# isl-org/Open3D-ML

Measured on AMD Instinct MI355X. Metric: point-cloud frames/sec (RandLA-Net SemanticKITTI inference: H2D + kNN pyramid + forward), higher is better.
Workload: dtype f32

## Files before the change

### open3d-ml_amd/csrc/randla.hip

```cpp
#include <hip/hip_runtime.h>
#include <math.h>
#include <stdint.h>
#include <stdlib.h>

#include <type_traits>

#include "gemm.h"
#include <gfx950_ops.h>
#include "grid.h"
#include "ml3d_hip.h"

namespace ml3d {

static int64_t fuse_rows() {
#ifdef ML3D_TEST_HOOKS
    static const int64_t rows = [] { const char* e = getenv("ML3D_RANDLA_FUSE_ROWS"); return e ? (int64_t)atoll(e) : (int64_t)64 * 1024; }();
    return rows;
#else
    return 64 * 1024;
#endif
}

#ifndef ML3D_ATTN_B3
#define ML3D_ATTN_B3 3
// ... 110 lines not shown
        if (m0 + r < A.m_total) {
            float v = acc[r];
            if (A.act) v = lrelu(v, A.slope);
            A.out[(m0 + r) * A.cout + o] = v;
        }
    }
}

struct LfaArgs {
    const float* xyz;
    const int32_t* nidx;
    int64_t n, n0, m_total;
    const float* gfeat;
    const float* lse1_wt;
    const float* lse1_b;
    const float* lse2_wt;
    const float* lse2_b;
    const float* score_wt;
    const float* score_b;
    const float* pool_wt;
    const float* pool_b;
    const float* mlp2_wt;
    const float* mlp2_b;
    const float* short_wt;
    const float* short_b;
    const float* feat_in;
    int d_in;
    float* out;
    int64_t xcd_chunk;
    const float* gscore;
    const int32_t* order;
};

__device__ __forceinline__ int64_t xcd_tile(int64_t i, int xcd, int64_t chunk, int64_t tiles) {
    const int64_t ci = i / chunk;
    const int64_t c = ci * 8 + xcd;
    if (c * chunk >= tiles) return -1;
    return c * chunk + (i - ci * chunk);
}

static int64_t xcd_chunk_tiles(int64_t tiles, int64_t batch) {
    if (batch <= 0 || tiles < 64) return 0;
    int64_t nch = batch;
    while (nch < 32) nch *= 2;
    int64_t chunk = (tiles + nch - 1) / nch;
    return chunk > 0 ? chunk : 0;
}

template <int D>
struct LfaCfg {
    static constexpr int H = D / 2;
    static constexpr int TP = (LFA_THREADS / D) > 0 ? (LFA_THREADS / D) : 1;
    static constexpr int CPT = D > LFA_THREADS ? D / LFA_THREADS : 1;
    static constexpr int CT = D > LFA_THREADS ? LFA_THREADS : D;
    static constexpr int XSLAB = D * XROW + 4;
};

template <int D>
__device__ __forceinline__ float attentive_pool(const float* Xp, int c, const float* __restrict__ score_wt,
                                                float bias) {
    float acc[RK];
#pragma unroll
    for (int k = 0; k < RK; ++k) acc[k] = bias;
    for (int j = 0; j < D; ++j) {
        float w = score_wt[j * D + c];
        const float4* xr = reinterpret_cast<const float4*>(Xp + j * XROW);
#pragma unroll
        for (int q = 0; q < RK / 4; ++q) {
            float4 x = xr[q];
            acc[4 * q + 0] = fmaf(x.x, w, acc[4 * q + 0]);
            acc[4 * q + 1] = fmaf(x.y, w, acc[4 * q + 1]);
            acc[4 * q + 2] = fmaf(x.z, w, acc[4 * q + 2]);
            acc[4 * q + 3] = fmaf(x.w, w, acc[4 * q + 3]);
        }
    }
    float mx = acc[0];
#pragma unroll
    for (int k = 1; k < RK; ++k) mx = fmaxf(mx, acc[k]);
    float sum = 0.f, agg = 0.f;
// ... 2197 lines not shown
}

template <class F>
static int dispatch_width(int dd, F f) {
    switch (dd) {
        case 8: return f(std::integral_constant<int, 8>{});
        case 16: return f(std::integral_constant<int, 16>{});
        case 32: return f(std::integral_constant<int, 32>{});
        case 64: return f(std::integral_constant<int, 64>{});
        case 128: return f(std::integral_constant<int, 128>{});
        case 256: return f(std::integral_constant<int, 256>{});
        case 512: return f(std::integral_constant<int, 512>{});
        default: return ML3D_E_UNSUPPORTED;
    }
}

__global__ void __launch_bounds__(256)
gather_max(const float* __restrict__ feat, const int32_t* __restrict__ nidx, float* __restrict__ out,
           int64_t n_in, int64_t n_out, int64_t batch, int c) {
    int64_t e = (int64_t)blockIdx.x * blockDim.x + threadIdx.x;
    if (e >= batch * n_out * c) return;
    int ch = (int)(e % c);
    int64_t r = e / c;
    int64_t b = r / n_out, i = r - b * n_out;
    const int32_t* id = nidx + (b * n_in + i) * RK;
    float v = -__builtin_inff();
#pragma unroll
    for (int k = 0; k < RK; ++k) v = fmaxf(v, feat[(b * n_in + id[k]) * c + ch]);
    out[r * c + ch] = v;
}

__global__ void __launch_bounds__(256)
gather_max4(const float* __restrict__ feat, const int32_t* __restrict__ nidx, float* __restrict__ out, uint32_t n_in,
            uint32_t n_out, uint32_t cv , uint32_t rows_per_block, const int32_t* __restrict__ order) {
    const uint32_t rl = threadIdx.x / cv, q = threadIdx.x - rl * cv;
    const uint32_t j = blockIdx.x * rows_per_block + rl;
    if (rl >= rows_per_block || j >= n_out) return;
    const uint32_t b = blockIdx.y;
    const uint32_t i = order ? (uint32_t)order[(size_t)b * n_out + j] - b * n_out : j;
    const int32_t* id = nidx + ((size_t)b * n_in + i) * RK;
    const float4* base = reinterpret_cast<const float4*>(feat + (size_t)b * n_in * (4 * cv)) + q;
    const float ninf = -__builtin_inff();
    float4 v = make_float4(ninf, ninf, ninf, ninf);
#pragma unroll
    for (int k = 0; k < RK; ++k) {
        const float4 x = base[(uint32_t)id[k] * cv];
        v.x = fmaxf(v.x, x.x); v.y = fmaxf(v.y, x.y); v.z = fmaxf(v.z, x.z); v.w = fmaxf(v.w, x.w);
    }
    reinterpret_cast<float4*>(out + ((size_t)b * n_out + i) * (4 * cv))[q] = v;
}

__global__ void __launch_bounds__(256)
gather_max_adjoint(const float* __restrict__ feat, const int32_t* __restrict__ nidx, const float* __restrict__ gout,
                   float* __restrict__ gfeat, int64_t n_in, int64_t n_out, int64_t batch, int c) {
    const int64_t e = (int64_t)blockIdx.x * blockDim.x + threadIdx.x;
    if (e >= batch * n_out * c) return;
    const int ch = (int)(e % c);
    const int64_t r = e / c;
    const int64_t b = r / n_out, i = r - b * n_out;
    const int32_t* id = nidx + (b * n_in + i) * RK;
    int64_t arg = b * n_in + id[0];
    float v = feat[arg * c + ch];
#pragma unroll
    for (int k = 1; k < RK; ++k) {
        const int64_t row = b * n_in + id[k];
        const float x = feat[row * c + ch];
        if (x > v) { v = x; arg = row; }
    }
    atomicAdd(gfeat + arg * c + ch, gout[r * c + ch]);
}

constexpr int AP_KMAX = 32;
template <bool BWD>
__global__ void __launch_bounds__(256)
attentive_pool_k(const float* __restrict__ scores, const float* __restrict__ x, const float* __restrict__ out_saved,
                 const float* __restrict__ gout, int64_t rows, int k, int c, float* __restrict__ out,
                 float* __restrict__ gscores, float* __restrict__ gx) {
    const int64_t e = (int64_t)blockIdx.x * blockDim.x + threadIdx.x;
    if (e >= rows * c) return;
    const int ch = (int)(e % c);
    const int64_t r = e / c;
    const float* sp = scores + r * k * c + ch;
// ... 291 lines not shown
            LfaArgs q1 = s1; q1.out = agg;
            const bool epi16 = dd == 16 && d_in == 8;
            if (epi16) q1.out = p1;
            const bool split = dd >= 32 && dd <= 256 && M * dd * 4 < ((int64_t)1 << 32) && M < ((int64_t)1 << 30);
            const bool b3_attn = ((ML3D_ATTN_B3) & 1) != 0 && split && ((dd == 128 && n[l] >= B3Cfg<128, 1>::TP) || (dd == 256 && n[l] >= B3Cfg<256, 1>::TP));
            auto point_scores = [&](const float* gfeat, int score_w, int score_b) {
                return run(8 * l + 7, lin(gfeat, h, score_w, (dd <= 64 || b3_attn) ? score_b : -1, p2, M, dd, 0.f));
            };
            if (split) { rc = point_scores(f1, sb + 4, sb + 5); if (rc) return rc; q1.gscore = p2; }
            rc = T.traced(8 * l + 1, [&] {
                return dispatch_width(dd, [&](auto w) { return launch_attn<decltype(w)::value, 1>(q1, st, epi16); });
            });
            if (rc) return rc;
            if (!epi16) {
                rc = run(8 * l + 4, lin(agg, dd, sb + 6, sb + 7, p1, M, h, 0.2f));
                if (rc) return rc;
            }
            LfaArgs q2 = s2; q2.out = epi16 ? enc : agg;
            if (split) { rc = point_scores(p1, sb + 10, sb + 11); if (rc) return rc; q2.gscore = p2; }
            rc = T.traced(8 * l + 2, [&] {
                return dispatch_width(dd, [&](auto w) { return launch_attn<decltype(w)::value, 2>(q2, st, epi16); });
            });
            if (rc) return rc;
            if (!epi16) {
                const LinArgs pool2[2] = {lin(agg, dd, sb + 12, sb + 13, p2, M, dd, 0.2f),
                                          lin(p2, dd, sb + 14, sb + 16, enc, M, 2 * dd, 0.01f, feat, d_in, sb + 17)};
                rc = launch_linears(pool2, 2, M >= fuse_rows(), T, 8 * l + 5, st);
            }
        } else {
            rc = dispatch_width(dd, [&](auto w) { return launch_lfa<decltype(w)::value>(s1, s2, st, T, 8 * l + 1); });
        }
        if (rc) return rc;
        rc = T.traced(8 * l + 3, [&] {
            const int c2 = 2 * dd;
            if ((c2 & 3) == 0 && c2 / 4 <= 256 && n[l] * c2 < ((int64_t)1 << 32) && B < 65536) {
                const uint32_t cv = (uint32_t)(c2 / 4), rpb = 256u / cv;
                const int32_t* ord = (tile_order && l + 1 < Lr) ? tile_order[l + 1] : nullptr;
                hipLaunchKernelGGL(gather_max4, dim3((unsigned)((n[l + 1] + rpb - 1) / rpb), (unsigned)B), dim3(256), 0, st, enc,
                                   neighbor_idx[l], samp, (uint32_t)n[l], (uint32_t)n[l + 1], cv, rpb, ord);
            } else {
                const int64_t items = B * n[l + 1] * c2;
                hipLaunchKernelGGL(gather_max, dim3((unsigned)((items + 255) / 256)), dim3(256), 0, st, enc,
                                   neighbor_idx[l], samp, n[l], n[l + 1], B, c2);
            }
            return hipGetLastError() == hipSuccess ? 0 : ML3D_E_LAUNCH;
        });
        if (rc) return rc;
        if (l == 0) enc_keep[0] = enc;
        enc_keep[l + 1] = samp;
        feat = samp;
        d_in = 2 * dd;
    }
    int slot = 2 + 18 * Lr;
    const int Dm = d_in;
    float* cur = take(B * n[Lr] * Dm);
    rc = run(1001, lin(feat, Dm, slot, slot + 1, cur, B * n[Lr], Dm, 0.2f));
    if (rc) return rc;
    slot += 2;
    auto fc1 = [&, fs = slot + 2 * Lr](LinArgs* g, const float* in, int k, float* t0, float* t1) {
        g[0] = lin(in, k, fs, fs + 1, t0, B * n[0], 64, 0.2f);
        g[1] = lin(t0, 64, fs + 2, fs + 3, t1, B * n[0], 32, 0.2f);
        g[2] = lin(t1, 32, fs + 4, fs + 5, out_scores, B * n[0], d->num_classes, 0.f);
    };
    int ed[ML3D_RANDLA_MAX_LAYERS + 1];
    enc_dims(d, ed);
    int cprev = Dm;
    for (int i = 0; i < Lr; ++i) {
        const int lev = Lr - 1 - i;
        const int skip_c = ed[Lr + 1 - i - 2];
        float* outp = take(B * n[lev] * skip_c);
        LinArgs a = lin(enc_keep[Lr + 1 - i - 2], skip_c, slot, slot + 1, outp, B * n[lev], skip_c, 0.2f, cur, cprev);
        a.gather = interp_idx[lev]; a.rows_per_item = n[lev]; a.a1_rows_per_item = n[lev + 1];
        if (i == Lr - 1) {
            LinArgs g[4] = {a};
            fc1(g + 1, outp, skip_c, nullptr, nullptr);
            const ChainArgs ch = chain_of(g, 4);
            if (mlp_shape_matches<ShapeDecFc1>(ch)) return T.traced(1200, [&] { return launch_chain_auto(ch, st); });
        }
        if (n[lev] >= 64 && (skip_c & 3) == 0 && (cprev & 3) == 0 && skip_c >= 8) {
            float* up = take(B * n[lev + 1] * skip_c);
            rc = T.traced(1100 + i, [&] {
                RowsA Au = {};
                Au.a = cur; Au.lda = cprev; Au.k1 = cprev;
                const int r = gemm_rows(Au, a.wt + (int64_t)skip_c * skip_c, B * n[lev + 1], skip_c, cprev, Epilogue{}, up, skip_c, nullptr, 0, st);
                if (r) return r;
                RowsA As = {};
                As.a = a.a0; As.lda = skip_c; As.k1 = skip_c;
                const Epilogue e1 = Epilogue::of(a.bias, 1, 0.2f).residual_rows(up, skip_c).gathered_residual(a.gather, 0, n[lev + 1], n[lev], n[lev + 1]);
                return gemm_rows(As, a.wt, a.m_total, skip_c, skip_c, e1, outp, skip_c, nullptr, 0, st);
            });
        } else {
            rc = run(1100 + i, a);
        }
        if (rc) return rc;
        slot += 2;
        cur = outp;
        cprev = skip_c;
    }
    float* t0 = take(B * n[0] * 64);
    float* t1 = take(B * n[0] * 32);
    LinArgs g[3];
    fc1(g, cur, cprev, t0, t1);
    return launch_linears(g, 3, true, T, 1200, st);
}

extern "C" int ml3d_randla_gather_max(const float* features, const int32_t* pool_idx, int64_t batch, int64_t n_in, int64_t n_out,
                                      int channels, float* out, void* stream) {
    if (batch < 0 || n_in < 0 || n_out < 0 || n_out > n_in || channels <= 0) return ML3D_E_INVALID;
    if (batch * n_out == 0) return 0;
    if (!features || !pool_idx || !out) return ML3D_E_INVALID;
    const int64_t total = batch * n_out * channels;
    hipLaunchKernelGGL(gather_max, dim3((unsigned)((total + 255) / 256)), dim3(256), 0, (hipStream_t)stream, features, pool_idx, out,
                       n_in, n_out, batch, channels);
    return hipGetLastError() == hipSuccess ? 0 : ML3D_E_LAUNCH;
}

extern "C" int ml3d_randla_gather_max_backward(const float* features, const int32_t* pool_idx, const float* grad_out, int64_t batch,
                                               int64_t n_in, int64_t n_out, int channels, float* grad_features, void* stream) {
    if (batch < 0 || n_in < 0 || n_out < 0 || n_out > n_in || channels <= 0) return ML3D_E_INVALID;
    if (batch * n_in == 0) return 0;
    if (!grad_features) return ML3D_E_INVALID;
    hipStream_t st = (hipStream_t)stream;
    if (hipMemsetAsync(grad_features, 0, sizeof(float) * (size_t)(batch * n_in) * (size_t)channels, st) != hipSuccess) return ML3D_E_LAUNCH;
    if (n_out == 0) return 0;
    if (!features || !pool_idx || !grad_out) return ML3D_E_INVALID;
    const int64_t total = batch * n_out * channels;
    hipLaunchKernelGGL(gather_max_adjoint, dim3((unsigned)((total + 255) / 256)), dim3(256), 0, st, features, pool_idx, grad_out,
                       grad_features, n_in, n_out, batch, channels);
    return hipGetLastError() == hipSuccess ? 0 : ML3D_E_LAUNCH;
}

extern "C" int ml3d_randla_attentive_pool(const float* scores, const float* x, int64_t rows, int k, int channels, float* out,
                                          void* stream) {
    if (rows < 0 || k <= 0 || channels <= 0) return ML3D_E_INVALID;
    if (k > AP_KMAX) return ML3D_E_UNSUPPORTED;
    if (rows == 0) return 0;
    if (!scores || !x || !out) return ML3D_E_INVALID;
    const int64_t total = rows * channels;
    hipLaunchKernelGGL((attentive_pool_k<false>), dim3((unsigned)((total + 255) / 256)), dim3(256), 0, (hipStream_t)stream, scores, x,
                       nullptr, nullptr, rows, k, channels, out, nullptr, nullptr);
    return hipGetLastError() == hipSuccess ? 0 : ML3D_E_LAUNCH;
}

extern "C" int ml3d_randla_attentive_pool_backward(const float* scores, const float* x, const float* out, const float* grad_out,
                                                   int64_t rows, int k, int channels, float* grad_scores, float* grad_x,
                                                   void* stream) {
    if (rows < 0 || k <= 0 || channels <= 0) return ML3D_E_INVALID;
// ... 9 lines not shown
```

### open3d-ml_amd/csrc/grid.h

```cpp
#pragma once
#include <hip/hip_runtime.h>
#include <stdint.h>

namespace ml3d {

constexpr int GRID_CAP = 8;
constexpr int GRID_SLACK = 64;
constexpr int GRID_LEVELS = 5;

struct Segs {
    const int64_t* splits;
    int64_t stride;
    int64_t n_uniform;
    int batch;
};

struct GridSeg {
    float lo[3];
    float c, inv_c;
    float margin;
    int dims[3];
    int cell_base;
    int n;
    int sorted_base;
    float c0;
    int dims0[3];
    float ext[3];
    float dim_est;
    int probe_stride;
};

struct GridView {
    const GridSeg* segs;
    const int* cell_start;
    const float4* sorted;
    int batch;
};

struct GridWs {
    GridSeg* segs;
    unsigned* bbox;
    unsigned* occ;
    unsigned* bitmap;
    int* cells;
    int* block_sums;
    float4* sorted;
    int64_t total_cells;
    int64_t bitmap_words;
    int64_t n_total;
    int batch;
};

constexpr int GRID_SORTED_SLACK = 4;
size_t grid_ws_bytes(int64_t n_total, int64_t batch);
bool grid_ws_carve(void* ws, size_t bytes, int64_t n_total, int64_t batch, GridWs* out);
int grid_build(const float* points, Segs segs, const GridWs& ws, float target_occ, hipStream_t stream);
int grid_build_derived(const float* points, Segs segs, const GridWs& ws, const GridWs& parent, hipStream_t stream);
int grid_build_fixed(const float* points, Segs segs, const GridWs& ws, float cell, hipStream_t stream);
int bbox_compute(const float* points, Segs segs, int64_t n_total, unsigned* bbox, unsigned* occ_scratch,
                 hipStream_t stream);
int scan_inclusive_i32(int* a, int64_t n, int* block_sums, hipStream_t stream);

void zero_async(void* ptr, size_t bytes, hipStream_t stream);

static inline char* ws_align(void* ws) { return (char*)(((uintptr_t)ws + 255) & ~(uintptr_t)255); }
static inline size_t ws_avail(const void* ws, size_t bytes) { return ws && bytes > 256 ? bytes - 256 : 0; }

__device__ __forceinline__ unsigned f2ord(float f) {
    unsigned u = __float_as_uint(f);
    return (u & 0x80000000u) ? ~u : (u | 0x80000000u);
}
__device__ __forceinline__ float ord2f(unsigned u) {
    return __uint_as_float((u & 0x80000000u) ? (u & 0x7fffffffu) : ~u);
}

__device__ __forceinline__ void wave_sync() {
    __threadfence_block();
    __builtin_amdgcn_wave_barrier();
}

__device__ __forceinline__ void wave_lds_sync() {
    __builtin_amdgcn_fence(__ATOMIC_RELEASE, "wavefront");
    __builtin_amdgcn_wave_barrier();
    __builtin_amdgcn_fence(__ATOMIC_ACQUIRE, "wavefront");
}


__device__ __forceinline__ float fmax_raw(float a, float b) { return __builtin_amdgcn_fmed3f(a, b, 3.0e38f); }

__device__ __forceinline__ int wave_inclusive_scan(int v) {
// ... 95 lines not shown
```

### open3d-ml_amd/csrc/grid.hip

```cpp
#include "grid.h"

#include <math.h>

namespace ml3d {

static inline size_t align_up(size_t x) { return (x + 255) & ~(size_t)255; }

static void grid_sizes(int64_t n_total, int64_t batch, int64_t* total_cells, int64_t* bitmap_words,
                       int64_t* n_blocks) {
    *total_cells = (int64_t)GRID_CAP * n_total + (int64_t)GRID_SLACK * batch;
    *bitmap_words = (*total_cells + 31) / 32 + batch;
    *n_blocks = (*total_cells + 2 + 1023) / 1024 + 1;
}

size_t grid_ws_bytes(int64_t n_total, int64_t batch) {
    int64_t tc, bw, nb;
    grid_sizes(n_total, batch, &tc, &bw, &nb);
    size_t b = 0;
    b += align_up(sizeof(GridSeg) * (size_t)batch);
    b += align_up(sizeof(unsigned) * 6 * (size_t)batch);
    b += align_up(sizeof(unsigned) * GRID_LEVELS * (size_t)batch);
    b += align_up(sizeof(unsigned) * GRID_LEVELS * (size_t)bw);
    b += align_up(sizeof(int) * (size_t)(tc + 2));
    b += align_up(sizeof(int) * (size_t)nb);
// ... 427 lines not shown
    for (int r = 0; r < 16; ++r) {
        int incl = wave_inclusive_scan(v[r]) + carry;
        int64_t i = base + r * 64 + lane;
        if (i < n) a[i] = incl;
        carry = __shfl(incl, 63);
    }
}

constexpr int SCAN_ONE_MAX = 32768;

__global__ void __launch_bounds__(1024) scan_one(int* a, int n) {
    __shared__ int ws[16];
    const int lane = threadIdx.x & 63, wv = threadIdx.x >> 6;
    const int rows = (n + 1023) / 1024;
    const int base = wv * rows * 64;
    int tot = 0;
    for (int r = 0; r < rows; ++r) {
        const int i = base + r * 64 + lane;
        if (i < n) tot += a[i];
    }
    tot = wave_sum(tot);
    if (lane == 0) ws[wv] = tot;
    __syncthreads();
    int carry = 0;
    for (int w = 0; w < wv; ++w) carry += ws[w];
    for (int r = 0; r < rows; ++r) {
        const int i = base + r * 64 + lane;
        const int incl = wave_inclusive_scan(i < n ? a[i] : 0) + carry;
        if (i < n) a[i] = incl;
        carry = __shfl(incl, 63);
    }
}

__global__ void grid_scatter(const float* __restrict__ pts, Segs S, int64_t n_total,
                             const GridSeg* __restrict__ segs, int* cells, float4* sorted) {
    int64_t i = (int64_t)blockIdx.x * blockDim.x + threadIdx.x;
    if (i >= n_total) return;
    int s; int64_t local;
    seg_locate(S, i, s, local);
    const float* p = pts + 3 * (seg_begin_global(S, s) + local);
    float x = p[0], y = p[1], z = p[2];
    int cid = point_cell(&segs[s], x, y, z);
    int pos = atomicAdd(&cells[cid + 1], 1);
    sorted[pos] = make_float4(x, y, z, __int_as_float((int)local));
}

__global__ void __launch_bounds__(256) grid_zero(uint4* __restrict__ p, size_t n16, uint32_t* __restrict__ tail, int ntail) {
    const size_t i = (size_t)blockIdx.x * blockDim.x + threadIdx.x;
    const size_t step = (size_t)gridDim.x * blockDim.x;
    for (size_t j = i; j < n16; j += step) p[j] = make_uint4(0u, 0u, 0u, 0u);
    if (i < (size_t)ntail) tail[i] = 0u;
}

void zero_async(void* ptr, size_t bytes, hipStream_t stream) {
    if (bytes == 0) return;
    if ((((uintptr_t)ptr) & 15) || (bytes & 3)) { (void)hipMemsetAsync(ptr, 0, bytes, stream); return; }
    const size_t n16 = bytes / 16;
    const int ntail = (int)((bytes - 16 * n16) / 4);
    const size_t want = (n16 + 255) / 256;
    const unsigned nb = (unsigned)(want < 1 ? 1 : (want > 2048 ? 2048 : want));
    hipLaunchKernelGGL(grid_zero, dim3(nb), dim3(256), 0, stream, (uint4*)ptr, n16, (uint32_t*)((char*)ptr + 16 * n16), ntail);
}

#define ML3D_LAUNCH_CHECK()                         \
    do {                                            \
        if (hipGetLastError() != hipSuccess) return -3; \
    } while (0)

int scan_inclusive_i32(int* a, int64_t n, int* block_sums, hipStream_t stream) {
    if (n <= 0) return 0;
    if (n <= SCAN_ONE_MAX) {
        hipLaunchKernelGGL(scan_one, dim3(1), dim3(1024), 0, stream, a, (int)n);
        ML3D_LAUNCH_CHECK();
        return 0;
    }
    int sbk = (int)((n + SCAN_TILE - 1) / SCAN_TILE);
    hipLaunchKernelGGL(scan_block_sums, dim3(sbk), dim3(256), 0, stream, a, n, block_sums);
    ML3D_LAUNCH_CHECK();
    hipLaunchKernelGGL(scan_sums, dim3(1), dim3(1024), 0, stream, block_sums, (int64_t)sbk);
    ML3D_LAUNCH_CHECK();
    hipLaunchKernelGGL(scan_final, dim3(sbk), dim3(256), 0, stream, a, n, block_sums);
    ML3D_LAUNCH_CHECK();
    return 0;
}

static int grid_sort(const float* points, Segs S, const GridWs& ws, hipStream_t stream) {
    int64_t n = ws.n_total;
    int nb = (int)((n + 255) / 256);
    if (n > 0) {
        hipLaunchKernelGGL(grid_hist, dim3(nb), dim3(256), 0, stream, points, S, n, ws.segs, ws.cells);
        ML3D_LAUNCH_CHECK();
        if (scan_inclusive_i32(ws.cells + 2, ws.total_cells, ws.block_sums, stream)) return -3;
        hipLaunchKernelGGL(grid_scatter, dim3(nb), dim3(256), 0, stream, points, S, n, ws.segs, ws.cells,
                           ws.sorted);
        ML3D_LAUNCH_CHECK();
    }
    return 0;
}


int grid_build(const float* points, Segs S, const GridWs& ws, float target_occ, hipStream_t stream) {
    int64_t n = ws.n_total;
    int B = ws.batch;
    if (B <= 0) return 0;
    if (target_occ <= 0.f) target_occ = 4.0f;
    int sb = (B + 63) / 64;
    zero_async(ws.bitmap, (size_t)((char*)(ws.cells + ws.total_cells + 2) - (char*)ws.bitmap), stream);
    hipLaunchKernelGGL(grid_bbox_init, dim3(sb), dim3(64), 0, stream, ws.bbox, ws.occ, B);
    ML3D_LAUNCH_CHECK();
    if (n > 0) {
        int nb4 = (int)((n + 1023) / 1024);
        hipLaunchKernelGGL(grid_bbox, dim3(nb4), dim3(256), 0, stream, points, S, n, ws.bbox);
        ML3D_LAUNCH_CHECK();
    }
    hipLaunchKernelGGL(grid_setup0, dim3(sb), dim3(64), 0, stream, S, ws.bbox, ws.segs, B);
    ML3D_LAUNCH_CHECK();
    int nb = (int)((n + 255) / 256);
    if (n > 0) {
        const int dense = (!S.splits && S.n_uniform >= 32768) ? 16 : 0;
        const int nbo = dense ? (int)((((S.n_uniform + dense - 1) / dense) * (int64_t)S.batch + 255) / 256) : nb;
        hipLaunchKernelGGL(grid_occupancy, dim3(nbo), dim3(256), 0, stream, points, S, n, ws.segs, ws.bitmap,
                           ws.bitmap_words, ws.occ, dense);
        ML3D_LAUNCH_CHECK();
    }
    hipLaunchKernelGGL(grid_setup1, dim3(sb), dim3(64), 0, stream, ws.occ, ws.segs, B, target_occ);
    ML3D_LAUNCH_CHECK();
    return grid_sort(points, S, ws, stream);
}

__global__ void grid_setup_fixed(GridSeg* segs, int batch, float cell) {
    int s = blockIdx.x * blockDim.x + threadIdx.x;
    if (s >= batch) return;
    GridSeg g = segs[s];
    float c = cell;
    if (!(c > 0.f)) c = g.c0;
    if (c < g.c0 * 0.5f) c = g.c0 * 0.5f;
    finish_grid(g, c, (int64_t)GRID_CAP * g.n + GRID_SLACK);
    segs[s] = g;
}

int bbox_compute(const float* points, Segs S, int64_t n, unsigned* bbox, unsigned* occ_scratch, hipStream_t stream) {
    int B = S.batch;
    if (B <= 0) return 0;
    hipLaunchKernelGGL(grid_bbox_init, dim3((B + 63) / 64), dim3(64), 0, stream, bbox, occ_scratch, B);
    ML3D_LAUNCH_CHECK();
    if (n > 0) {
        hipLaunchKernelGGL(grid_bbox, dim3((unsigned)((n + 1023) / 1024)), dim3(256), 0, stream, points, S, n, bbox);
        ML3D_LAUNCH_CHECK();
    }
    return 0;
}

int grid_build_fixed(const float* points, Segs S, const GridWs& ws, float cell, hipStream_t stream) {
    int B = ws.batch;
    if (B <= 0) return 0;
    int sb = (B + 63) / 64;
    zero_async(ws.cells, sizeof(int) * (size_t)(ws.total_cells + 2), stream);
    if (bbox_compute(points, S, ws.n_total, ws.bbox, ws.occ, stream)) return -3;
    hipLaunchKernelGGL(grid_setup0, dim3(sb), dim3(64), 0, stream, S, ws.bbox, ws.segs, B);
    ML3D_LAUNCH_CHECK();
    hipLaunchKernelGGL(grid_setup_fixed, dim3(sb), dim3(64), 0, stream, ws.segs, B, cell);
    ML3D_LAUNCH_CHECK();
    return grid_sort(points, S, ws, stream);
}

int grid_build_derived(const float* points, Segs S, const GridWs& ws, const GridWs& parent, hipStream_t stream) {
    int B = ws.batch;
    if (B <= 0) return 0;
    zero_async(ws.cells, sizeof(int) * (size_t)(ws.total_cells + 2), stream);
    hipLaunchKernelGGL(grid_setup_derived, dim3((B + 63) / 64), dim3(64), 0, stream, S, parent.segs, ws.segs, B);
    ML3D_LAUNCH_CHECK();
    return grid_sort(points, S, ws, stream);
}

}
```

### open3d-ml_amd/csrc/knn.hip

```cpp
#include <hip/hip_runtime.h>
#include <stdint.h>
#include <stdlib.h>

#include <gfx950_ops.h>

#include "grid.h"
#include "ml3d_hip.h"

namespace ml3d {

typedef unsigned long long u64;
constexpr u64 KEY_EMPTY = 0x7ff0000000000000ull;

struct QuerySrc {
    const float4* sorted_q;
    const GridSeg* qsegs;
    const float* raw;
    Segs segs;
    int64_t n_total;
};

template <int K>
__device__ __forceinline__ void topk_insert(double (&best)[K], double key) {
    if (key < best[K - 1]) {
// ... 324 lines not shown
        hipLaunchKernelGGL((knn_first<16, SUB>), dim3(blocks), dim3(T), 0, stream, J, k, index_local, vec, H);
        if (hipGetLastError() != hipSuccess) return ML3D_E_LAUNCH;
        hipLaunchKernelGGL((knn_continue<16, SUB>), dim3((H.cap + T - 1) / T), dim3(T), 0, stream, J, k, index_local, vec, H);
        return hipGetLastError() == hipSuccess ? 0 : ML3D_E_LAUNCH;
    }
    if (k == 1) hipLaunchKernelGGL((knn_query_multi<1, SUB, false>), dim3(blocks), dim3(T), 0, stream, J, k, index_local, vec, H);
    else if (k <= 8) hipLaunchKernelGGL((knn_query_multi<8, SUB, false>), dim3(blocks), dim3(T), 0, stream, J, k, index_local, vec, H);
    else if (k <= 16) hipLaunchKernelGGL((knn_query_multi<16, SUB, false>), dim3(blocks), dim3(T), 0, stream, J, k, index_local, vec, H);
    else if (k <= 32) hipLaunchKernelGGL((knn_query_multi<32, SUB, false>), dim3(blocks), dim3(T), 0, stream, J, k, index_local, vec, H);
    else if (k <= 64) hipLaunchKernelGGL((knn_query_multi<64, SUB, false>), dim3(blocks), dim3(T), 0, stream, J, k, index_local, vec, H);
    else return ML3D_E_UNSUPPORTED;
    return hipGetLastError() == hipSuccess ? 0 : ML3D_E_LAUNCH;
}

static int launch_query(const GridView& G, const QuerySrc& Q, int k, int index_local, Segs support_segs,
                        int32_t* out_idx, float* out_d2, hipStream_t stream) {
    if (Q.n_total <= 0) return 0;
    dim3 grid((unsigned)((Q.n_total + 255) / 256)), block(256);
    if (k == 1)
        hipLaunchKernelGGL(knn_query<1>, grid, block, 0, stream, G, Q, k, index_local, support_segs, out_idx, out_d2);
    else if (k <= 8)
        hipLaunchKernelGGL(knn_query<8>, grid, block, 0, stream, G, Q, k, index_local, support_segs, out_idx, out_d2);
    else if (k <= 16)
        hipLaunchKernelGGL(knn_query<16>, grid, block, 0, stream, G, Q, k, index_local, support_segs, out_idx, out_d2);
    else if (k <= 32)
        hipLaunchKernelGGL(knn_query<32>, grid, block, 0, stream, G, Q, k, index_local, support_segs, out_idx, out_d2);
    else if (k <= 64)
        hipLaunchKernelGGL(knn_query<64>, grid, block, 0, stream, G, Q, k, index_local, support_segs, out_idx, out_d2);
    else
        return ML3D_E_UNSUPPORTED;
    return hipGetLastError() == hipSuccess ? 0 : ML3D_E_LAUNCH;
}

__global__ void order_from_grid(const float4* __restrict__ sorted, int64_t n_total, int64_t n_per_item,
                                int32_t* __restrict__ out) {
    const int64_t i = (int64_t)blockIdx.x * blockDim.x + threadIdx.x;
    if (i >= n_total) return;
    out[i] = (int32_t)((i / n_per_item) * n_per_item + (int64_t)__float_as_int(sorted[i].w));
}

static constexpr float tuning_occ() { return 0.f; }

}

using namespace ml3d;

extern "C" int ml3d_abi_version(void) { return ML3D_ABI_VERSION; }

extern "C" size_t ml3d_knn_workspace_bytes(int64_t n_points, int64_t n_queries, int64_t batch) {
    (void)n_queries;
    return grid_ws_bytes(n_points, batch);
}

extern "C" int ml3d_knn_search(const float* points, const int64_t* points_row_splits, const float* queries,
                               const int64_t* queries_row_splits, int64_t batch, int64_t n_points,
                               int64_t n_queries, int k, int index_local, int32_t* out_index,
                               float* out_dist2, void* workspace, size_t workspace_bytes, void* stream) {
    if (!points_row_splits || !queries_row_splits || batch <= 0 || k <= 0 || n_points < 0 || n_queries < 0 ||
        n_points > 0x7fffffffll / GRID_CAP - 4096 || n_queries > 0x7fffffffll)
        return ML3D_E_INVALID;
    if (k > 64) return ML3D_E_UNSUPPORTED;
    if (n_queries == 0) return 0;
    if (!out_index || (n_points > 0 && !points) || !queries) return ML3D_E_INVALID;
    GridWs ws;
    if (!grid_ws_carve(workspace, workspace_bytes, n_points, batch, &ws)) return ML3D_E_WORKSPACE;
    hipStream_t st = (hipStream_t)stream;
    Segs ps = {points_row_splits, 0, 0, (int)batch};
    Segs qs = {queries_row_splits, 0, 0, (int)batch};
    int rc = grid_build(points, ps, ws, tuning_occ(), st);
    if (rc) return ML3D_E_LAUNCH;
    GridView G = grid_view(ws);
    QuerySrc Q;
    bool self = (queries == points) && (queries_row_splits == points_row_splits) && (n_queries == n_points);
// ... 41 lines not shown
    return ml3d_randla_knn_pyramid_ordered(points, batch, n0, num_layers, ratios_host, k, neighbor_idx_host,
                                           interp_idx_host, nullptr, workspace, workspace_bytes, stream, tr);
}

extern "C" int ml3d_randla_knn_pyramid_ordered(const float* points, int64_t batch, int64_t n0, int num_layers,
                                               const int32_t* ratios_host, int k,
                                               int32_t* const* neighbor_idx_host, int32_t* const* interp_idx_host,
                                               int32_t* const* tile_order_host, void* workspace,
                                               size_t workspace_bytes, void* stream, const ml3d_trace* tr) {
    auto tb = [&](int tag) { for (const ml3d_trace* r = tr; r; r = r->next) if (r->tag == tag && r->ev_start) (void)hipEventRecord((hipEvent_t)r->ev_start, (hipStream_t)stream); };
    auto te = [&](int tag) { for (const ml3d_trace* r = tr; r; r = r->next) if (r->tag == tag && r->ev_stop) (void)hipEventRecord((hipEvent_t)r->ev_stop, (hipStream_t)stream); };
    if (!points || batch <= 0 || n0 <= 0 || num_layers <= 0 || num_layers > KNN_MAX_JOBS || !ratios_host || k <= 0 ||
        !neighbor_idx_host || !interp_idx_host)
        return ML3D_E_INVALID;
    if (k > 64) return ML3D_E_UNSUPPORTED;
    int64_t n[17];
    if (pyramid_sizes(n0, num_layers, ratios_host, n)) return ML3D_E_INVALID;
    if (n0 * batch > 0x7fffffffll / GRID_CAP - 4096) return ML3D_E_INVALID;
    if (workspace_bytes < ml3d_randla_pyramid_workspace_bytes(batch, n0, num_layers, ratios_host))
        return ML3D_E_WORKSPACE;
    hipStream_t st = (hipStream_t)stream;
    GridWs ws[17];
    char* p = (char*)workspace;
    for (int l = 0; l < num_layers; ++l) {
        size_t bytes = grid_ws_bytes(n[l] * batch, batch) + 256;
        if (!grid_ws_carve(p, bytes, n[l] * batch, batch, &ws[l])) return ML3D_E_WORKSPACE;
        p += bytes;
    }
    float occ = tuning_occ();
    for (int l = 0; l < num_layers; ++l) {
        if (n[l] == 0) continue;
        Segs S = {nullptr, n0, n[l], (int)batch};
        tb(100 + l);
        if (l == 0 ? grid_build(points, S, ws[l], occ, st) : grid_build_derived(points, S, ws[l], ws[0], st))
            return ML3D_E_LAUNCH;
        if (tile_order_host && tile_order_host[l]) {
            const int64_t nt = n[l] * batch;
            hipLaunchKernelGGL(order_from_grid, dim3((unsigned)((nt + 255) / 256)), dim3(256), 0, st, ws[l].sorted, nt, n[l],
                               tile_order_host[l]);
            if (hipGetLastError() != hipSuccess) return ML3D_E_LAUNCH;
        }
        te(100 + l);
    }
    KnnJobs Jk;
    Jk.n = 0;
    for (int l = 0; l < num_layers; ++l) {
        if (n[l] == 0) continue;
        Segs S = {nullptr, n0, n[l], (int)batch};
        QuerySrc Q;
        Q.sorted_q = ws[l].sorted;
        Q.qsegs = ws[l].segs;
        Q.raw = points;
        Q.segs = S;
        Q.n_total = n[l] * batch;
        KnnJob& a = Jk.j[Jk.n++];
        a.G = grid_view(ws[l]); a.Q = Q; a.support = S; a.out_idx = neighbor_idx_host[l]; a.block_begin = 0;
        a.out_sub = interp_idx_host[l];
        a.n_sub = (int)n[l + 1];
    }
    int64_t total_q = 0;
    for (int l = 0; l < num_layers; ++l) total_q += n[l] * batch;
    const Handoff hand = handoff_carve(p, total_q);
    tb(0);
    int rc = launch_query_multi<true>(Jk, k, 1, st, &hand);
    te(0);
    return rc;
}

#include <hip/hip_fp16.h>

#include "patchloop.h"
#include "sort.h"

namespace ml3d {
// ... 248 lines not shown
```

Before: 7474.

## Split pooling gather into L2-sized channel slabs with XCD-aware block mapping

The random-sampling max-pool gather now divides the channel dimension into slabs sized so that one slab of the input feature map fits in a 2 MiB L2 budget. Blocks are remapped so that each XCD processes contiguous chunks of a single (batch, slab) unit. The aim is to keep gathered neighbour rows resident in each XCD's L2 rather than re-reading them from HBM. The public gather_max entry point also moves to the vectorised path when alignment allows. This adds index arithmetic per block, and narrower slabs make each thread's loads less contiguous.

After: 7496 (median of 2 runs). About the same (+0.3%).

```diff
diff --git a/open3d-ml_amd/csrc/randla.hip b/open3d-ml_amd/csrc/randla.hip
--- a/open3d-ml_amd/csrc/randla.hip
+++ b/open3d-ml_amd/csrc/randla.hip
@@ -166,9 +166,10 @@
     const int32_t* order;
 };
 
-__device__ __forceinline__ int64_t xcd_tile(int64_t i, int xcd, int64_t chunk, int64_t tiles) {
-    const int64_t ci = i / chunk;
-    const int64_t c = ci * 8 + xcd;
+template <class I>
+__device__ __forceinline__ I xcd_tile(I i, int xcd, I chunk, I tiles) {
+    const I ci = i / chunk;
+    const I c = ci * 8 + xcd;
     if (c * chunk >= tiles) return -1;
     return c * chunk + (i - ci * chunk);
 }
@@ -179,6 +180,30 @@
     while (nch < 32) nch *= 2;
     int64_t chunk = (tiles + nch - 1) / nch;
     return chunk > 0 ? chunk : 0;
+}
+
+constexpr int64_t POOL_L2_BUDGET = (int64_t)2 << 20;
+struct PoolPlan {
+    int w;
+    int rpb;
+    int64_t chunk, split;
+    unsigned grid;
+};
+static PoolPlan pool_plan(int64_t B, int64_t n_in, int64_t n_out, int c, bool ordered) {
+    const PoolPlan plain = {c, 256 / (c / 4), 0, 1, 0};
+    int w = c;
+    if (c % 32 == 0 && c > 32) {
+        w = 32;
+        for (int x = 64; x <= c; x += 32)
+            if (c % x == 0 && n_in * x * 4 <= POOL_L2_BUDGET) w = x;
+    }
+    const int64_t slabs = c / w, rpb = 256 / (w / 4), rb = (n_out + rpb - 1) / rpb;
+    if (B * slabs < 8 || (ordered && c <= 32)) return plain;
+    int64_t split = 1;
+    while (B * slabs * split < 32) split *= 2;
+    const int64_t chunk = (rb + split - 1) / split, nch = B * slabs * split;
+    if (nch * chunk + 8 * chunk >= ((int64_t)1 << 31)) return plain;
+    return PoolPlan{w, (int)rpb, chunk, split, (unsigned)(8 * ((nch + 7) / 8 * chunk))};
 }
 
 template <int D>
@@ -2442,14 +2467,24 @@
 
 __global__ void __launch_bounds__(256)
 gather_max4(const float* __restrict__ feat, const int32_t* __restrict__ nidx, float* __restrict__ out, uint32_t n_in,
-            uint32_t n_out, uint32_t cv , uint32_t rows_per_block, const int32_t* __restrict__ order) {
-    const uint32_t rl = threadIdx.x / cv, q = threadIdx.x - rl * cv;
-    const uint32_t j = blockIdx.x * rows_per_block + rl;
+            uint32_t n_out, uint32_t cv , uint32_t wv , uint32_t rows_per_block,
+            const int32_t* __restrict__ order, uint32_t batch, int32_t xcd_chunk, int32_t split) {
+    const uint32_t rl = threadIdx.x / wv, q = threadIdx.x - rl * wv;
+    uint32_t b = blockIdx.y, jb = blockIdx.x, q0 = 0;
+    if (xcd_chunk > 0) {
+        const int32_t rb = (int32_t)((n_out + rows_per_block - 1) / rows_per_block);
+        const int32_t per_cs = split * xcd_chunk, slabs = (int32_t)(cv / wv), units = (int32_t)batch * slabs * per_cs;
+        const int32_t t = xcd_tile<int32_t>((int32_t)(blockIdx.x >> 3), (int)(blockIdx.x & 7), xcd_chunk, units);
+        if (t < 0 || t >= units) return;
+        const int32_t cs = t / per_cs, r = t - cs * per_cs;
+        if (r >= rb) return;
+        b = (uint32_t)(cs / slabs); jb = (uint32_t)r; q0 = ((uint32_t)cs - b * (uint32_t)slabs) * wv;
+    }
+    const uint32_t j = jb * rows_per_block + rl;
     if (rl >= rows_per_block || j >= n_out) return;
-    const uint32_t b = blockIdx.y;
     const uint32_t i = order ? (uint32_t)order[(size_t)b * n_out + j] - b * n_out : j;
     const int32_t* id = nidx + ((size_t)b * n_in + i) * RK;
-    const float4* base = reinterpret_cast<const float4*>(feat + (size_t)b * n_in * (4 * cv)) + q;
+    const float4* base = reinterpret_cast<const float4*>(feat + (size_t)b * n_in * (4 * cv)) + q0 + q;
     const float ninf = -__builtin_inff();
     float4 v = make_float4(ninf, ninf, ninf, ninf);
 #pragma unroll
@@ -2457,7 +2492,22 @@
         const float4 x = base[(uint32_t)id[k] * cv];
         v.x = fmaxf(v.x, x.x); v.y = fmaxf(v.y, x.y); v.z = fmaxf(v.z, x.z); v.w = fmaxf(v.w, x.w);
     }
-    reinterpret_cast<float4*>(out + ((size_t)b * n_out + i) * (4 * cv))[q] = v;
+    reinterpret_cast<float4*>(out + ((size_t)b * n_out + i) * (4 * cv))[q0 + q] = v;
+}
+
+static int launch_pool(const float* feat, const int32_t* idx, float* out, int64_t n_in, int64_t n_out, int64_t B, int c,
+                       const int32_t* order, hipStream_t st) {
+    const bool aligned = (((uintptr_t)feat | (uintptr_t)out) & 15) == 0;
+    if ((c & 3) == 0 && c / 4 <= 256 && n_in * c < ((int64_t)1 << 32) && B < 65536 && aligned) {
+        const PoolPlan p = pool_plan(B, n_in, n_out, c, order != nullptr);
+        const dim3 grid = p.chunk ? dim3(p.grid) : dim3((unsigned)((n_out + p.rpb - 1) / p.rpb), (unsigned)B);
+        hipLaunchKernelGGL(gather_max4, grid, dim3(256), 0, st, feat, idx, out, (uint32_t)n_in, (uint32_t)n_out, (uint32_t)(c / 4),
+                           (uint32_t)(p.w / 4), (uint32_t)p.rpb, order, (uint32_t)B, (int32_t)p.chunk, (int32_t)p.split);
+    } else {
+        const int64_t items = B * n_out * c;
+        hipLaunchKernelGGL(gather_max, dim3((unsigned)((items + 255) / 256)), dim3(256), 0, st, feat, idx, out, n_in, n_out, B, c);
+    }
+    return hipGetLastError() == hipSuccess ? 0 : ML3D_E_LAUNCH;
 }
 
 __global__ void __launch_bounds__(256)
@@ -2815,18 +2865,8 @@
         }
         if (rc) return rc;
         rc = T.traced(8 * l + 3, [&] {
-            const int c2 = 2 * dd;
-            if ((c2 & 3) == 0 && c2 / 4 <= 256 && n[l] * c2 < ((int64_t)1 << 32) && B < 65536) {
-                const uint32_t cv = (uint32_t)(c2 / 4), rpb = 256u / cv;
-                const int32_t* ord = (tile_order && l + 1 < Lr) ? tile_order[l + 1] : nullptr;
-                hipLaunchKernelGGL(gather_max4, dim3((unsigned)((n[l + 1] + rpb - 1) / rpb), (unsigned)B), dim3(256), 0, st, enc,
-                                   neighbor_idx[l], samp, (uint32_t)n[l], (uint32_t)n[l + 1], cv, rpb, ord);
-            } else {
-                const int64_t items = B * n[l + 1] * c2;
-                hipLaunchKernelGGL(gather_max, dim3((unsigned)((items + 255) / 256)), dim3(256), 0, st, enc,
-                                   neighbor_idx[l], samp, n[l], n[l + 1], B, c2);
-            }
-            return hipGetLastError() == hipSuccess ? 0 : ML3D_E_LAUNCH;
+            const int32_t* ord = (tile_order && l + 1 < Lr) ? tile_order[l + 1] : nullptr;
+            return launch_pool(enc, neighbor_idx[l], samp, n[l], n[l + 1], B, 2 * dd, ord, st);
         });
         if (rc) return rc;
         if (l == 0) enc_keep[0] = enc;
@@ -2892,10 +2932,7 @@
     if (batch < 0 || n_in < 0 || n_out < 0 || n_out > n_in || channels <= 0) return ML3D_E_INVALID;
     if (batch * n_out == 0) return 0;
     if (!features || !pool_idx || !out) return ML3D_E_INVALID;
-    const int64_t total = batch * n_out * channels;
-    hipLaunchKernelGGL(gather_max, dim3((unsigned)((total + 255) / 256)), dim3(256), 0, (hipStream_t)stream, features, pool_idx, out,
-                       n_in, n_out, batch, channels);
-    return hipGetLastError() == hipSuccess ? 0 : ML3D_E_LAUNCH;
+    return launch_pool(features, pool_idx, out, n_in, n_out, batch, channels, nullptr, (hipStream_t)stream);
 }
 
 extern "C" int ml3d_randla_gather_max_backward(const float* features, const int32_t* pool_idx, const float* grad_out, int64_t batch,
```

## Scan and zero only used per-item grid cells; emit tile order in scatter

Applied to the files above, without the earlier changes.

For uniform per-item batches, the grid build now zeros only the cells each segment actually uses and runs a segmented two-pass scan over each item's cell range. Previously it zeroed and scanned the full worst-case cell table. The separate order_from_grid kernel is removed, and the tile order is written directly by grid_scatter. This cuts memory traffic and kernel launches in the kNN pyramid build, at the cost of more complex indexing and new segment-boundary edge cases in the per-item scan.

Result: no change. 7637 before, 7565 after (-0.9%).

```diff
diff --git a/open3d-ml_amd/csrc/grid.h b/open3d-ml_amd/csrc/grid.h
--- a/open3d-ml_amd/csrc/grid.h
+++ b/open3d-ml_amd/csrc/grid.h
@@ -54,8 +54,9 @@
 constexpr int GRID_SORTED_SLACK = 4;
 size_t grid_ws_bytes(int64_t n_total, int64_t batch);
 bool grid_ws_carve(void* ws, size_t bytes, int64_t n_total, int64_t batch, GridWs* out);
-int grid_build(const float* points, Segs segs, const GridWs& ws, float target_occ, hipStream_t stream);
-int grid_build_derived(const float* points, Segs segs, const GridWs& ws, const GridWs& parent, hipStream_t stream);
+int grid_build(const float* points, Segs segs, const GridWs& ws, float target_occ, hipStream_t stream, int32_t* order = nullptr);
+int grid_build_derived(const float* points, Segs segs, const GridWs& ws, const GridWs& parent, hipStream_t stream,
+                       int32_t* order = nullptr);
 int grid_build_fixed(const float* points, Segs segs, const GridWs& ws, float cell, hipStream_t stream);
 int bbox_compute(const float* points, Segs segs, int64_t n_total, unsigned* bbox, unsigned* occ_scratch,
                  hipStream_t stream);
diff --git a/open3d-ml_amd/csrc/grid.hip b/open3d-ml_amd/csrc/grid.hip
--- a/open3d-ml_amd/csrc/grid.hip
+++ b/open3d-ml_amd/csrc/grid.hip
@@ -483,8 +483,70 @@
     }
 }
 
+__device__ __forceinline__ int seg_ncells(const GridSeg* g) { return g->dims[0] * g->dims[1] * g->dims[2]; }
+
+__global__ void __launch_bounds__(256)
+seg_scan_tile_sums(const GridSeg* __restrict__ segs, const int* __restrict__ cells, int* __restrict__ block_sums) {
+    __shared__ int ws[4];
+    const int s = blockIdx.y;
+    const GridSeg* g = &segs[s];
+    const int ncells = seg_ncells(g);
+    const int base = blockIdx.x * SCAN_TILE;
+    if (base >= ncells) return;
+    const int* a = cells + (int64_t)g->cell_base + 2;
+    int v = 0;
+#pragma unroll
+    for (int j = 0; j < SCAN_TILE / 256; ++j) {
+        const int i = base + j * 256 + threadIdx.x;
+        if (i < ncells) v += a[i];
+    }
+    v = wave_sum(v);
+    if ((threadIdx.x & 63) == 0) ws[threadIdx.x >> 6] = v;
+    __syncthreads();
+    if (threadIdx.x == 0) block_sums[(int64_t)s * gridDim.x + blockIdx.x] = ws[0] + ws[1] + ws[2] + ws[3];
+}
+
+__global__ void __launch_bounds__(256)
+seg_scan_final(const GridSeg* __restrict__ segs, int* cells, const int* __restrict__ block_sums) {
+    __shared__ int ws[4], ps[4];
+    const int lane = threadIdx.x & 63, wv = threadIdx.x >> 6;
+    const int s = blockIdx.y, t = blockIdx.x;
+    const GridSeg* g = &segs[s];
+    const int ncells = seg_ncells(g);
+    if (t * SCAN_TILE >= ncells) return;
+    int* a = cells + (int64_t)g->cell_base + 2;
+    int before = 0;
+    for (int j = threadIdx.x; j < t; j += 256) before += block_sums[(int64_t)s * gridDim.x + j];
+    before = wave_sum(before);
+    const int base = t * SCAN_TILE + wv * 1024;
+    int v[16], tot = 0;
+#pragma unroll
+    for (int r = 0; r < 16; ++r) {
+        const int i = base + r * 64 + lane;
+        v[r] = i < ncells ? a[i] : 0;
+        tot += v[r];
+    }
+    tot = wave_sum(tot);
+    if (lane == 0) { ws[wv] = tot; ps[wv] = before; }
+    __syncthreads();
+    int carry = s * g->n + ps[0] + ps[1] + ps[2] + ps[3];
+    for (int w = 0; w < wv; ++w) carry += ws[w];
+#pragma unroll
+    for (int r = 0; r < 16; ++r) {
+        const int incl = wave_inclusive_scan(v[r]) + carry;
+        const int i = base + r * 64 + lane;
+        if (i < ncells) a[i] = incl;
+        carry = __shfl(incl, 63);
+    }
+    if ((t + 1) * SCAN_TILE >= ncells && wv == 3 && lane == 0) {
+        const int cap = GRID_CAP * g->n + GRID_SLACK;
+        if (cap - 2 >= ncells) a[cap - 2] = carry;
+        if (cap - 1 >= ncells) a[cap - 1] = carry;
+    }
+}
+
 __global__ void grid_scatter(const float* __restrict__ pts, Segs S, int64_t n_total,
-                             const GridSeg* __restrict__ segs, int* cells, float4* sorted) {
+                             const GridSeg* __restrict__ segs, int* cells, float4* sorted, int32_t* __restrict__ order) {
     int64_t i = (int64_t)blockIdx.x * blockDim.x + threadIdx.x;
     if (i >= n_total) return;
     int s; int64_t local;
@@ -494,6 +556,7 @@
     int cid = point_cell(&segs[s], x, y, z);
     int pos = atomicAdd(&cells[cid + 1], 1);
     sorted[pos] = make_float4(x, y, z, __int_as_float((int)local));
+    if (order) order[pos] = (int32_t)(seg_begin_packed(S, s) + local);
 }
 
 __global__ void __launch_bounds__(256) grid_zero(uint4* __restrict__ p, size_t n16, uint32_t* __restrict__ tail, int ntail) {
@@ -513,6 +576,25 @@
     hipLaunchKernelGGL(grid_zero, dim3(nb), dim3(256), 0, stream, (uint4*)ptr, n16, (uint32_t*)((char*)ptr + 16 * n16), ntail);
 }
 
+__global__ void __launch_bounds__(256) grid_zero_used(const GridSeg* __restrict__ segs, int* __restrict__ cells) {
+    const int s = blockIdx.y;
+    const GridSeg* g = &segs[s];
+    const int lo = s == 0 ? 0 : 2, hi = 2 + seg_ncells(g);
+    const int w0 = blockIdx.x * SCAN_TILE;
+    if (w0 >= hi) return;
+    int* base = cells + (int64_t)g->cell_base;
+#pragma unroll
+    for (int j = 0; j < SCAN_TILE / 1024; ++j) {
+        const int w = w0 + 4 * (j * 256 + threadIdx.x);
+        if (w >= lo && w + 4 <= hi) {
+            *(uint4*)(base + w) = make_uint4(0u, 0u, 0u, 0u);
+        } else {
+            for (int k = 0; k < 4; ++k)
+                if (w + k >= lo && w + k < hi) base[w + k] = 0;
+        }
+    }
+}
+
 #define ML3D_LAUNCH_CHECK()                         \
     do {                                            \
         if (hipGetLastError() != hipSuccess) return -3; \
@@ -535,28 +617,51 @@
     return 0;
 }
 
-static int grid_sort(const float* points, Segs S, const GridWs& ws, hipStream_t stream) {
+static inline bool per_item_table(const Segs& S, const GridWs& ws) {
+    return !S.splits && S.n_uniform > 0 && ws.batch > 0 && ws.batch <= 65535 && ws.n_total == S.n_uniform * (int64_t)ws.batch;
+}
+static inline unsigned tiles_of(int64_t words) { return (unsigned)((words + SCAN_TILE - 1) / SCAN_TILE); }
+
+static int zero_used_cells(const Segs& S, const GridWs& ws, hipStream_t stream) {
+    const int64_t cap = (int64_t)GRID_CAP * S.n_uniform + GRID_SLACK;
+    hipLaunchKernelGGL(grid_zero_used, dim3(tiles_of(cap + 2), (unsigned)ws.batch), dim3(256), 0, stream, ws.segs, ws.cells);
+    ML3D_LAUNCH_CHECK();
+    return 0;
+}
+
+static int grid_sort(const float* points, Segs S, const GridWs& ws, hipStream_t stream, int32_t* order) {
     int64_t n = ws.n_total;
     int nb = (int)((n + 255) / 256);
     if (n > 0) {
         hipLaunchKernelGGL(grid_hist, dim3(nb), dim3(256), 0, stream, points, S, n, ws.segs, ws.cells);
         ML3D_LAUNCH_CHECK();
-        if (scan_inclusive_i32(ws.cells + 2, ws.total_cells, ws.block_sums, stream)) return -3;
+        if (per_item_table(S, ws)) {
+            const dim3 grid(tiles_of((int64_t)GRID_CAP * S.n_uniform + GRID_SLACK), (unsigned)ws.batch);
+            if (grid.x > 1) {
+                hipLaunchKernelGGL(seg_scan_tile_sums, grid, dim3(256), 0, stream, ws.segs, ws.cells, ws.block_sums);
+                ML3D_LAUNCH_CHECK();
+            }
+            hipLaunchKernelGGL(seg_scan_final, grid, dim3(256), 0, stream, ws.segs, ws.cells, ws.block_sums);
+            ML3D_LAUNCH_CHECK();
+        } else if (scan_inclusive_i32(ws.cells + 2, ws.total_cells, ws.block_sums, stream)) {
+            return -3;
+        }
         hipLaunchKernelGGL(grid_scatter, dim3(nb), dim3(256), 0, stream, points, S, n, ws.segs, ws.cells,
-                           ws.sorted);
+                           ws.sorted, order);
         ML3D_LAUNCH_CHECK();
     }
     return 0;
 }
 
 
-int grid_build(const float* points, Segs S, const GridWs& ws, float target_occ, hipStream_t stream) {
+int grid_build(const float* points, Segs S, const GridWs& ws, float target_occ, hipStream_t stream, int32_t* order) {
     int64_t n = ws.n_total;
     int B = ws.batch;
     if (B <= 0) return 0;
     if (target_occ <= 0.f) target_occ = 4.0f;
     int sb = (B + 63) / 64;
-    zero_async(ws.bitmap, (size_t)((char*)(ws.cells + ws.total_cells + 2) - (char*)ws.bitmap), stream);
+    const bool per_item = per_item_table(S, ws);
+    zero_async(ws.bitmap, (size_t)((char*)(per_item ? ws.cells : ws.cells + ws.total_cells + 2) - (char*)ws.bitmap), stream);
     hipLaunchKernelGGL(grid_bbox_init, dim3(sb), dim3(64), 0, stream, ws.bbox, ws.occ, B);
     ML3D_LAUNCH_CHECK();
     if (n > 0) {
@@ -576,7 +681,8 @@
     }
     hipLaunchKernelGGL(grid_setup1, dim3(sb), dim3(64), 0, stream, ws.occ, ws.segs, B, target_occ);
     ML3D_LAUNCH_CHECK();
-    return grid_sort(points, S, ws, stream);
+    if (per_item && zero_used_cells(S, ws, stream)) return -3;
+    return grid_sort(points, S, ws, stream, order);
 }
 
 __global__ void grid_setup_fixed(GridSeg* segs, int batch, float cell) {
@@ -612,16 +718,18 @@
     ML3D_LAUNCH_CHECK();
     hipLaunchKernelGGL(grid_setup_fixed, dim3(sb), dim3(64), 0, stream, ws.segs, B, cell);
     ML3D_LAUNCH_CHECK();
-    return grid_sort(points, S, ws, stream);
-}
-
-int grid_build_derived(const float* points, Segs S, const GridWs& ws, const GridWs& parent, hipStream_t stream) {
+    return grid_sort(points, S, ws, stream, nullptr);
+}
+
+int grid_build_derived(const float* points, Segs S, const GridWs& ws, const GridWs& parent, hipStream_t stream, int32_t* order) {
     int B = ws.batch;
     if (B <= 0) return 0;
-    zero_async(ws.cells, sizeof(int) * (size_t)(ws.total_cells + 2), stream);
+    const bool per_item = per_item_table(S, ws);
+    if (!per_item) zero_async(ws.cells, sizeof(int) * (size_t)(ws.total_cells + 2), stream);
     hipLaunchKernelGGL(grid_setup_derived, dim3((B + 63) / 64), dim3(64), 0, stream, S, parent.segs, ws.segs, B);
     ML3D_LAUNCH_CHECK();
-    return grid_sort(points, S, ws, stream);
-}
-
-}
+    if (per_item && zero_used_cells(S, ws, stream)) return -3;
+    return grid_sort(points, S, ws, stream, order);
+}
+
+}
diff --git a/open3d-ml_amd/csrc/knn.hip b/open3d-ml_amd/csrc/knn.hip
--- a/open3d-ml_amd/csrc/knn.hip
+++ b/open3d-ml_amd/csrc/knn.hip
@@ -380,13 +380,6 @@
     return hipGetLastError() == hipSuccess ? 0 : ML3D_E_LAUNCH;
 }
 
-__global__ void order_from_grid(const float4* __restrict__ sorted, int64_t n_total, int64_t n_per_item,
-                                int32_t* __restrict__ out) {
-    const int64_t i = (int64_t)blockIdx.x * blockDim.x + threadIdx.x;
-    if (i >= n_total) return;
-    out[i] = (int32_t)((i / n_per_item) * n_per_item + (int64_t)__float_as_int(sorted[i].w));
-}
-
 static constexpr float tuning_occ() { return 0.f; }
 
 }
@@ -494,14 +487,9 @@
         if (n[l] == 0) continue;
         Segs S = {nullptr, n0, n[l], (int)batch};
         tb(100 + l);
-        if (l == 0 ? grid_build(points, S, ws[l], occ, st) : grid_build_derived(points, S, ws[l], ws[0], st))
+        int32_t* order = tile_order_host ? tile_order_host[l] : nullptr;
+        if (l == 0 ? grid_build(points, S, ws[l], occ, st, order) : grid_build_derived(points, S, ws[l], ws[0], st, order))
             return ML3D_E_LAUNCH;
-        if (tile_order_host && tile_order_host[l]) {
-            const int64_t nt = n[l] * batch;
-            hipLaunchKernelGGL(order_from_grid, dim3((unsigned)((nt + 255) / 256)), dim3(256), 0, st, ws[l].sorted, nt, n[l],
-                               tile_order_host[l]);
-            if (hipGetLastError() != hipSuccess) return ML3D_E_LAUNCH;
-        }
         te(100 + l);
     }
     KnnJobs Jk;
```
